# actapia/rna_clique

Hardware: AMD Instinct MI355X
Metric: sample-pairs/sec (all-vs-all alignment -> RBH graph -> distance matrix) (higher is better)
Workload: dtype u8/int32

## Files before the change

### include/rcgpu.h

```cpp
#ifndef RCGPU_H
#define RCGPU_H

#include <stdint.h>

#ifdef __cplusplus
extern "C" {
#endif

#define RC_OK 0
#define RC_E_ARG (-1)
#define RC_E_STATE (-2)
#define RC_E_HIP (-3)
#define RC_E_NOMEM (-4)
#define RC_E_NO_IDEAL (-5)
#define RC_E_CAPACITY (-6)
#define RC_E_LIMIT (-7)
#define RC_E_IO (-8)

typedef struct rc_engine rc_engine;

typedef struct rc_opts {
    int32_t top_matches;
    int32_t keep_all;
    double evalue;
// ... 66 lines not shown
    double dev_peak_bytes;
    double defer_length;
    double defer_gaveup;
    double defer_outside;
    double index_reused;
    double ext_retries;
    double load_ms;
    double align_wall_ms;
    double host_wait_ms;
    double later_seeds;
    double later_whole;
    double index_fb_ranges;
    double index_fb_keys;
    double resample_ms;
    double nj_ms;
} rc_timing;

void rc_default_opts(rc_opts *opts);

int rc_create(const rc_opts *opts, rc_engine **eng);
int rc_destroy(rc_engine *eng);
const char *rc_last_error(void);
void rc_dev_peak_reset(void);

int rc_add_sample(rc_engine *eng, const char *label, const char *seq,
                  const uint64_t *tx_offsets, const int32_t *gene,
                  const int32_t *iso, uint32_t n_tx, int32_t *sample_id);

int rc_add_hsps(rc_engine *eng, int32_t q, int32_t s, const rc_hsp *hsps, uint64_t n);

int rc_upload(rc_engine *eng);

int rc_run(rc_engine *eng);
int rc_align(rc_engine *eng);
int rc_finish(rc_engine *eng);

uint64_t rc_edge_record_size(void);
int rc_export_edges(rc_engine *eng, void *buf, uint64_t cap, uint64_t *n, int on_device);
// ... 75 lines not shown
```

### rna_clique_amd/_native.py

```python
from __future__ import annotations

import ctypes
import os
import sys

import numpy as np

HERE = os.path.dirname(os.path.abspath(__file__))
LIB_PATH = os.environ.get("RC_LIB") or os.path.join(HERE, "librcgpu.so")

RC_OK = 0
RC_E_ARG = -1
RC_E_STATE = -2
RC_E_HIP = -3
RC_E_NOMEM = -4
RC_E_NO_IDEAL = -5
RC_E_CAPACITY = -6
RC_E_LIMIT = -7


class RcOpts(ctypes.Structure):
    _fields_ = [("top_matches", ctypes.c_int32), ("keep_all", ctypes.c_int32),
                ("evalue", ctypes.c_double), ("word_size", ctypes.c_int32),
                ("xdrop_half", ctypes.c_int32), ("device", ctypes.c_int32),
# ... 43 lines not shown

EDGE_RECORD_DTYPE = np.dtype([("a", np.uint32), ("b", np.uint32), ("pair", np.uint32),
                              ("nident", np.int32), ("den", np.int32)])
RC_EDGE_SUM_ONLY = 0x80000000
RC_NODE_ONLY = 0x7FFFFFFF


class RcTiming(ctypes.Structure):
    _fields_ = [(n, ctypes.c_double) for n in (
        "pack_ms", "index_ms", "align_ms", "topn_ms", "rbh_ms", "graph_ms",
        "reduce_ms", "total_ms", "seed_kernel_ms", "align_kernel_ms", "ext_steps",
        "ext_calls", "ext_fullband", "ext_deferred", "big_passes", "tiles", "dust_ms",
        "band_bound", "maxhsp_bound", "ext_second", "near_index", "reverse_seeds", "ext_slides", "ext_wide", "dev_bytes",
        "dev_peak_bytes", "defer_length", "defer_gaveup", "defer_outside", "index_reused",
        "ext_retries", "load_ms", "align_wall_ms", "host_wait_ms", "later_seeds", "later_whole",
        "index_fb_ranges", "index_fb_keys", "resample_ms", "nj_ms")]


assert HSP_DTYPE.itemsize == ctypes.sizeof(RcHsp)
assert ROW_DTYPE.itemsize == ctypes.sizeof(RcRow)

P = ctypes.POINTER
VP = ctypes.c_void_p
SIGNATURES = {
    "rc_default_opts": (None, [P(RcOpts)]),
    "rc_create": (ctypes.c_int, [P(RcOpts), P(VP)]),
    "rc_destroy": (ctypes.c_int, [VP]),
    "rc_last_error": (ctypes.c_char_p, []),
    "rc_dev_peak_reset": (None, []),
    "rc_add_sample": (ctypes.c_int, [VP, ctypes.c_char_p, ctypes.c_char_p,
                                     P(ctypes.c_uint64), P(ctypes.c_int32),
                                     P(ctypes.c_int32), ctypes.c_uint32,
                                     P(ctypes.c_int32)]),
    "rc_add_hsps": (ctypes.c_int, [VP, ctypes.c_int32, ctypes.c_int32, VP, ctypes.c_uint64]),
    "rc_upload": (ctypes.c_int, [VP]),
    "rc_run": (ctypes.c_int, [VP]),
    "rc_align": (ctypes.c_int, [VP]),
    "rc_finish": (ctypes.c_int, [VP]),
    "rc_edge_record_size": (ctypes.c_uint64, []),
    "rc_export_edges": (ctypes.c_int, [VP, VP, ctypes.c_uint64, P(ctypes.c_uint64), ctypes.c_int]),
    "rc_import_edges": (ctypes.c_int, [VP, VP, ctypes.c_uint64, ctypes.c_int]),
    "rc_import_edge_parts": (ctypes.c_int, [VP, VP, VP, ctypes.c_int32, ctypes.c_uint64, ctypes.c_int]),
    "rc_trim": (ctypes.c_int, [VP]),
    "rc_set_sample_count": (ctypes.c_int, [VP, ctypes.c_int32]),
# ... 78 lines not shown
```

### rna_clique_amd/csrc/align.hip

```cpp
#include "device.h"

#include <algorithm>
#include <climits>
#include <cstdlib>
#include <type_traits>

namespace rcg {

constexpr int SBLOCK = 256;
#ifndef RC_SEED_CAP
#define RC_SEED_CAP 512
#endif
#ifndef RC_SEED_WAVES
#define RC_SEED_WAVES 5
#endif
constexpr int SEED_CAP = RC_SEED_CAP;
static_assert((SEED_CAP & (SEED_CAP - 1)) == 0, "RC_SEED_CAP must be a power of two");
#ifndef RC_HBATCH
#define RC_HBATCH 6
#endif
constexpr int HBATCH = RC_HBATCH;
#ifndef RC_SEED_REV_WAVES
#define RC_SEED_REV_WAVES 7
#endif
// ... 1431 lines not shown
__device__ __forceinline__ RowArgsK row_args()
{
    RowArgsK p = (RowArgsK)__builtin_amdgcn_kernarg_segment_ptr();
    asm volatile("" : "+s"(p));
    return p;
}

struct RowLds {
    int meta[RM_N];
    int st[RS_N];
};
enum { WM_GA0, WM_GB0, WM_AARR, WM_BARR, WM_ALO, WM_ALIM, WM_BLO, WM_BLIM, WM_W0, WM_N = WM_W0 + 4 };
struct RowWin {
    int w[WM_N];
};
__host__ __device__ constexpr size_t row_lds_bytes(int rw, int na, int sw, bool win = false)
{
    return ((size_t)(EBLOCK / rw) * na * sw + 2) * 8 + (NSHARD + 1) * 8 + (size_t)(EBLOCK / rw) * sizeof(RowLds) + 32 +
           (win ? (size_t)(EBLOCK / rw) * sizeof(RowWin) : 0);
}
constexpr int WIN_MARGIN = 48;

template <bool AMB, int RW, int MINW, bool SAVE = false, bool WIN = false>
__global__ __launch_bounds__(EBLOCK, MINW) void extend_rows_kernel(RowArgs)
{
    constexpr int RROWS = EBLOCK / RW;
    constexpr int RC0 = RW / 2;
    constexpr int NA = AMB ? 8 : 4;
    constexpr int EBIT = 26, OBIT = 13;
    extern __shared__ uint64_t rstg[];
    const int sw = row_args()->P.dsw;
    unsigned long long *const sprefix = reinterpret_cast<unsigned long long *>(rstg + 2 + (size_t)RROWS * NA * sw);
    RowLds *const rows_lds = reinterpret_cast<RowLds *>(sprefix + NSHARD + 1);
    uint32_t *const rcnt = reinterpret_cast<uint32_t *>(rows_lds + RROWS);
    uint32_t &s_ncand = rcnt[4];
    RowWin *const rows_win = reinterpret_cast<RowWin *>(rcnt + 8);
    {
        const RowArgsK K = row_args();
        if (threadIdx.x < 4 || threadIdx.x == 5) rcnt[threadIdx.x] = 0;
        for (int i = threadIdx.x; i <= NSHARD; i += EBLOCK) sprefix[i] = K->P.shard_prefix[i];
        if (threadIdx.x == 0) s_ncand = K->P.list ? (uint32_t)*K->P.list_n : (uint32_t)K->P.n_cand;
    }
    __syncthreads();

    const int lane = threadIdx.x & 63, rl = lane & (RW - 1), row = lane / RW;
    const int rs = threadIdx.x / RW;
    const int k = rl - RC0;
    uint64_t *stg = rstg + 2 + (size_t)rs * NA * sw;
    const uint32_t base0 = 4u * (uint32_t)reinterpret_cast<uintptr_t>(rstg) + (uint32_t)(2 + rs * NA * sw) * 32u;
    const uint32_t bqr = base0 + 64u * (uint32_t)sw, btr = bqr + 32u * (uint32_t)sw;
    const uint32_t moff = 128u * (uint32_t)sw;
    RowLds &RL = rows_lds[rs];
    int *meta = RL.meta;
    int *const wm = rows_win[rs].w;
    const int X = row_args()->P.xdrop;
    auto chunk = []() { return (uint32_t)max(row_args()->P.chunk, 1); };
    uint32_t lnx = 0;
    auto grab = [&]() {
        const uint32_t ncand = s_ncand, ch = chunk();
        unsigned long long b = 0;
        if (rl == 0) b = atomicAdd(row_args()->P.work, (unsigned long long)ch);
        b = (unsigned long long)__shfl((long long)b, RW * row);
        lnx = b < ncand ? (uint32_t)b : ncand;
        if (rl == 0) RL.st[RS_LEND] = (int)(lnx + ch);
    };
    auto slot = [&](uint32_t l, int which) -> uint64_t {
        int sh = RL.st[which];
        while (sh + 1 < NSHARD && sprefix[sh + 1] <= l) sh++;
        if (rl == 0) RL.st[which] = sh;
// ... 21 lines not shown
            } else if (wide && K->P.wide) {
                wi2 = atomicAdd(K->P.wide_n, 1ull);
                K->P.wide[wi2] = (uint32_t)ci;
            }
            box_out()[ci * BOX_REC + FX_STATUS] = -1;
        }
        if constexpr (SAVE) return (unsigned long long)__shfl((long long)wi2, RW * row);
        return wi2;
    };
    if (rl == 0) {
        RL.st[RS_SHARD] = 0;
        RL.st[RS_SHN] = 0;
    }
    grab();
    int recv = load_rec(lnx);

    int act = A_FETCH;
    int R = -1, goe = 0, wi = 0, wg = 0, wd = 0, best = 0, bl = RC0, d6 = 0;
    uint32_t pa = 0, pb = 0;
    int alen = 0, blen = 0;
    uint32_t pbk = 0;
    int blk = 0, nkd = 0;
    int mnk = 0;
    bool swap = false;
    int wlo = 0, wlim = 0;

    using GW = const __attribute__((address_space(1))) uint64_t *;
    auto warr = [](int arr, bool mask) -> GW {
        const RowArgsK K = row_args();
        GW f = (GW)(mask ? K->db.AF : K->db.F), r = (GW)(mask ? K->db.ARC : K->db.RC);
// ... 106 lines not shown
#endif
        int r0 = 0;
        if constexpr (WIN) {
            win_begin(done_act == A_LDONE ? 1 : 0);
            const int m0 = min(alen, blen);
            bool pend = false;
            if (rl == RC0) {
                const int mw = min(m0, wlim);
                r0 = slide_fwd<AMB>(pa, pb, max(mw, 0), moff);
                pend = mw < m0 && r0 >= mw;
            }
            if (ballot(pend)) win_resolve(0, r0, m0, pend);
        } else {
            if (rl == RC0) r0 = slide_fwd<AMB>(pa, pb, min(alen, blen), moff);
        }
        r0 = __shfl(r0, RW * row + RC0);
        best = 2 * r0;
        bl = RC0;
        if (rl == RC0) {
            wi = r0;
            wg = 0;
            wd = 0;
        }
        R = rl == RC0 ? r0 : -1;
        goe = 0;
        if (rl == 0 && d6) atomicAdd(&rcnt[5], (uint32_t)d6);
        d6 = 0;
        if constexpr (!WIN) pbk = pb - (uint32_t)k;
        blk = blen + k;
        mnk = max(min(alen, blk), 0);
        nkd = -k;
        if (rl == 0) {
            atomicAdd(&rcnt[0], 1u);
            meta[RM_PHASE] = done_act;
            meta[RM_KOF] = 0;
        }
        act = (min(alen, blen) - r0 <= 0) ? done_act : done_act + (A_STEP_R - A_RDONE);
#ifdef RC_ROW_TIMING
        t_ei += __builtin_readcyclecounter() - e0t;
#endif
    };

#ifdef RC_ROW_TIMING
    unsigned long long t_tr = 0, t_st = 0, t_fe = 0, t_sl = 0;
    unsigned long long n16 = 0, c16 = 0, sl16 = 0;
    bool ov16 = false, had = false;
    int w16 = 0;
#endif
    for (;;) {
#ifdef RC_ROW_TIMING
        const unsigned long long c0t = __builtin_readcyclecounter();
#endif
        while (act < A_DONE) {
            if (act == A_FETCH) {
#ifdef RC_ROW_TIMING
                const unsigned long long f0t = __builtin_readcyclecounter();
#endif
                if (lnx >= s_ncand) {
                    R = -1;
                    act = A_DONE;
                    continue;
                }
                const uint64_t ci = cslot(lnx, RS_SHARD);
#ifdef RC_ROW_TIMING
                if (rl == 0 && had && !ov16) c16++;
                ov16 = false;
                had = true;
#endif
                if (rl < CAND_DWORDS) meta[RM_REC + rl] = recv;
                if (rl == 0) {
                    meta[RM_CLO] = (int)(uint32_t)ci;
                    meta[RM_CHI] = (int)(uint32_t)(ci >> 32);
// ... 191 lines not shown
                    }
                    bl = BL_PARKED;
                }
                const int from = rl + s;
                const bool in = from >= 0 && from < RW;
                const int nR = __shfl(R, RW * row + (in ? from : rl)), ng = __shfl(goe, RW * row + (in ? from : rl));
                R = in ? nR : -1;
                goe = in ? ng : 0;
                pbk -= (uint32_t)s;
                blk += s;
                mnk = max(min(alen, blk), 0);
                nkd -= s;
                if constexpr (WIN) win_lane(k + kn);
                if (rl == 0) {
                    meta[RM_KOF] = kn;
                    atomicAdd(&rcnt[3], 1u);
                }
                __builtin_amdgcn_fence(__ATOMIC_RELEASE, "wavefront");
                __builtin_amdgcn_wave_barrier();
                act = meta[RM_PHASE] + (A_STEP_R - A_RDONE);
#ifdef RC_ROW_TIMING
                t_sl += __builtin_readcyclecounter() - s0t;
#endif
            } else if (act == A_RDONE || act == A_LDONE) {
                int ei, ed, ego, kb;
                if (bl == BL_PARKED) {
                    ei = meta[RM_PWI];
                    ed = meta[RM_PWD] / 6;
                    ego = meta[RM_PWG];
                    kb = meta[RM_PK];
                } else {
// ... 13 lines not shown
                        meta[RM_RI] = ei;
                        meta[RM_RJ] = ej;
                        meta[RM_RD] = ed;
                        meta[RM_RGO] = ego;
                    }
                    const int x = meta[RM_X], y = meta[RM_Y];
                    const int Lq = meta[RM_REC + RC_LQ], Lt = meta[RM_REC + RC_LT];
                    pa = (uint32_t)meta[RM_QB] + (uint32_t)(Lq - x);
                    alen = x;
                    pb = (uint32_t)meta[RM_TB] + (uint32_t)(Lt - y);
                    blen = y;
                    if (swap) {
                        const uint32_t t = pa; pa = pb; pb = t;
                        const int u = alen; alen = blen; blen = u;
                    }
                    ext_init(A_LDONE);
                } else {
                    const uint64_t ci = (uint64_t)(uint32_t)meta[RM_CLO] | ((uint64_t)(uint32_t)meta[RM_CHI] << 32);
                    int v = 0;
                    if (rl >= FX_R && rl < FX_R + 5) v = meta[RM_RSC + (rl - FX_R)];
                    if (rl == FX_L) v = best;
                    if (rl == FX_L + 1) v = ei;
                    if (rl == FX_L + 2) v = ej;
                    if (rl == FX_L + 3) v = ed;
                    if (rl == FX_L + 4) v = ego;
                    if (rl < BOX_REC) box_out()[ci * BOX_REC + rl] = v;
                    act = A_FETCH;
                }
            } else {
                const uint64_t ci = (uint64_t)(uint32_t)meta[RM_CLO] | ((uint64_t)(uint32_t)meta[RM_CHI] << 32);
                const unsigned long long wi2 = defer(ci, true);
                if constexpr (SAVE && RW == 32) {
                    if (wi2 != ~0ull) {
                        const RowArgsK K = row_args();
                        if (K->P.resume && wi2 < K->P.res_cap) {
                            int *rec = K->P.resume + (size_t)wi2 * RES_REC;
                            rec[RES_R + rl] = R;
                            rec[RES_G + rl] = goe;
                            if (rl <= RES_PK) rec[rl] = meta[RM_RSC + rl];
                            if (rl == RES_D6) rec[rl] = meta[RM_AD6];
                            if (rl == RES_BEST) rec[rl] = meta[RM_ABEST];
                        }
                    }
                }
                if (rl == 0) atomicAdd(&rcnt[2], 1u);
                act = A_FETCH;
            }
        }
#ifdef RC_ROW_TIMING
        const unsigned long long c1t = __builtin_readcyclecounter();
        t_tr += c1t - c0t;
#endif
        const bool ext = act >= A_STEP_R;
        const uint64_t mext = m_ge(act, A_STEP_R);
        if (!mext) break;
        if (ext) {
            d6 += 6;
            nkd -= 6;
            const int Rl = rw_from_lower<RW, true>(R, -1, rl), Rr = rw_from_upper<RW, true>(R, -1, rl);
            const int gl = rw_from_lower<RW, false>(goe, 0, rl), gr = rw_from_upper<RW, false>(goe, 0, rl);
// ... 86 lines not shown
            const uint64_t medge = RW == 64 ? 0ull : rw_spread<RW>(mlive & EDGES);
            act = lane_sel(mcont, lane_sel_k<A_SLIDE>(medge, act), act - (A_STEP_R - A_RDONE));
        }
#ifdef RC_ROW_TIMING
        t_st += __builtin_readcyclecounter() - c1t;
#endif
    }
#ifdef RC_ROW_TIMING
    unsigned long long *const counters = row_args()->P.counters;
    if (lane == 0 && counters) {
        atomicAdd(&counters[DC_T_TRANS - DC_COUNTERS], t_tr);
        atomicAdd(&counters[DC_T_STEPS - DC_COUNTERS], t_st);
        atomicAdd(&counters[DC_T_FETCH - DC_COUNTERS], t_fe);
        atomicAdd(&counters[DC_T_SLIDE - DC_COUNTERS], t_sl);
        atomicAdd(&counters[DC_T_START - DC_COUNTERS], t_ei);
    }
    if (rl == 0 && had && !ov16) c16++;
    if (rl == 0 && counters) {
        atomicAdd(&counters[DC_T_N16 - DC_COUNTERS], n16);
        atomicAdd(&counters[DC_T_C16 - DC_COUNTERS], c16);
        atomicAdd(&counters[DC_T_SL16 - DC_COUNTERS], sl16);
    }
#endif
    unsigned long long *const ctr = row_args()->P.counters;
    if (rl == 0 && d6) atomicAdd(&rcnt[5], (uint32_t)d6);
    __syncthreads();
    if (threadIdx.x < 4 && ctr) atomicAdd(&ctr[DC_EXTS - DC_COUNTERS + threadIdx.x], (unsigned long long)rcnt[threadIdx.x]);
    if (threadIdx.x == 5 && ctr) atomicAdd(&ctr[DC_STEPS - DC_COUNTERS], (unsigned long long)(rcnt[5] / 6u));
}

__global__ __launch_bounds__(256) void first_finish_kernel(ExtParams P)
{
    constexpr int OBIT = 13, GMASK = 8191;
    for (uint64_t li = blockIdx.x * (uint64_t)blockDim.x + threadIdx.x; li < P.n_cand;
         li += (uint64_t)gridDim.x * blockDim.x) {
        int lo = 0, hi = NSHARD;
        while (hi - lo > 1) {
            const int mid = (lo + hi) >> 1;
            if (P.shard_prefix[mid] <= li) lo = mid; else hi = mid;
        }
        const uint64_t ci = (uint64_t)lo * P.cand_cap + (li - P.shard_prefix[lo]);
// ... 572 lines not shown
    if (hipOccupancyMaxActiveBlocksPerMultiprocessor(&per_cu, kernel, EBLOCK, lds) != hipSuccess || per_cu < 1)
        per_cu = 1;
    return (unsigned)(cus * per_cu);
}

template <bool A, int RWV, bool SV, bool WV>
static void launch_rows_t(const Db &db, const ExtParams &P, hipStream_t st)
{
    auto kern = extend_rows_kernel<A, RWV, ROW_MIN_WAVES, SV, WV>;
    const size_t lds = row_lds_bytes(RWV, A ? 8 : 4, P.dsw, WV);
    hipLaunchKernelGGL(kern, dim3(resident_blocks(kern, lds)), dim3(EBLOCK), lds, st, RowArgs{db, P});
}
template <int RWV, bool SV = false>
static void launch_rows(bool amb, const Db &db, const ExtParams &P, hipStream_t st)
{
    if (amb) {
        if (P.win) launch_rows_t<true, RWV, SV, true>(db, P, st); else launch_rows_t<true, RWV, SV, false>(db, P, st);
    } else {
        if (P.win) launch_rows_t<false, RWV, SV, true>(db, P, st); else launch_rows_t<false, RWV, SV, false>(db, P, st);
    }
}

int row_slot_words_max(bool amb)
{
    const int na = amb ? 8 : 4, rows = EBLOCK / 32;
    const size_t per_block = (size_t)(160 * 1024) / (size_t)ROW_MIN_WAVES;
    const size_t fixed = row_lds_bytes(32, na, 0, true);
    return (int)((per_block - fixed) / ((size_t)rows * na * 8));
}

static void extend_lists(bool amb, const Db &db, const ExtParams &B, hipStream_t st)
{
    for (int dir = 0; dir < (B.share ? 2 : 1); dir++) {
        ExtParams W3 = B;
        W3.dir = dir;
        if (dir) {
            W3.defer = B.defer_r;
            W3.defer_count = B.defer_r_count;
        }
        if (amb) {
            auto kern = extend_kernel<true>;
            hipLaunchKernelGGL(kern, dim3(resident_blocks(kern, 0)), dim3(EBLOCK), 0, st, db, W3);
        } else {
// ... 147 lines not shown
```

### rna_clique_amd/csrc/device.h

```cpp
#pragma once
#include <hip/hip_runtime.h>
#include <stdint.h>

namespace rcg {

constexpr int W16 = 16;
constexpr int BAND = 64;
constexpr int BAND_LO = -32;
constexpr int MAX_HSP = 8;
constexpr int DMAX = 4096;
constexpr int ISO_LDS = 128;
constexpr uint64_t MAX_TX = 1ull << 27;
constexpr int MAX_SAMPLES = 65535;

struct TxInfo {
    uint64_t start;
    uint32_t len;
    int32_t sample;
};

__host__ __device__ __forceinline__ size_t grp_index(uint32_t gene, int sample, uint32_t n_genes)
{
    return (size_t)sample * n_genes + gene;
}
// ... 194 lines not shown
    DC_DEFER_R,
    DC_WORK3,
    DC_MBIG,
    DC_WIDE0,
    DC_WIDE1,
    DC_WORK_W0,
    DC_WORK_W1,
    DC_WHY,
    DC_WHY_END = DC_WHY + 3,
    DC_T_N16 = DC_WHY_END,
    DC_T_FETCH,
    DC_T_SLIDE,
    DC_T_START,
    DC_T_C16,
    DC_T_SL16,
    DC_N = 32
};
static_assert(DC_DEFER == DC_COUNTERS + 5 && DC_WORK == DC_COUNTERS + 6, "defer_count and work alias counters[5], [6]");
static_assert(DC_COUNTERS_END == 12 && DC_WHY == 22 && DC_T_SL16 == 30 && DC_T_SL16 < DC_N, "d_count layout");

struct ExtParams {
    int32_t xdrop;
    int32_t sym;
    int32_t max_len;
    const int32_t *thr;
    const int32_t *bits10;
    const Cand *cands;
    const GSeed *seeds;
    const unsigned long long *shard_prefix;
    uint64_t n_cand;
    uint64_t cand_cap;
    DHsp *cand_hsp;
    uint8_t *cand_nh;
    uint32_t *cand_ovf;
    DHsp *ovf;
    uint64_t ovf_cap;
    unsigned long long *ovf_count;
    unsigned int *status;
    unsigned long long *counters;
    int32_t dsw;
    int32_t win;
    int32_t *cand_box;
    int32_t chunk;
    unsigned long long *work;
    uint32_t *defer;
    unsigned long long *defer_count;
    const uint32_t *list;
    const unsigned long long *list_n;
    int32_t share;
    int32_t which;
    int32_t dir;
    int32_t *cand_box2;
    DHsp *cand_hsp_r;
    uint8_t *cand_nh_r;
    uint32_t *cand_ovf_r;
    uint32_t *defer_r;
// ... 180 lines not shown
```

### rna_clique_amd/csrc/engine.hip

```cpp
#include "../../include/rcgpu.h"
#include "device.h"
#include "graph_pickle.h"

#include <cstring>
#include <rocprim/device/device_radix_sort.hpp>
#include <rocprim/device/device_scan.hpp>
#include <rocprim/iterator/counting_iterator.hpp>

#include <algorithm>
#include <cmath>
#include <cstdio>
#include <cstdlib>
#include <cstring>
#include <array>
#include <atomic>
#include <chrono>
#include <condition_variable>
#include <deque>
#include <functional>
#include <map>
#include <memory>
#include <mutex>
#include <numeric>
#include <string>
// ... 42 lines not shown
void launch_near_fill(bool, const TxInfo *, uint32_t, const uint8_t *, const uint64_t *, const uint64_t *,
                      const uint64_t *, uint64_t *, uint64_t, unsigned long long *, hipStream_t);
void launch_seed(bool, const Db &, const Index &, const SeedParams &, hipStream_t);
void launch_seed_big(bool, const Db &, const Index &, const SeedParams &, uint32_t, hipStream_t);
void launch_rs_range(const uint32_t *, uint32_t, uint32_t, uint32_t, uint32_t *, hipStream_t);
void launch_dust(bool, uint64_t, uint64_t, const uint64_t *, const uint64_t *, const uint64_t *, const TxInfo *, uint32_t, int,
                 int, int, uint32_t *, uint64_t *, uint32_t, uint64_t *, hipStream_t);
uint32_t dust_scratch_words(uint32_t);
uint64_t dust_event_words(uint32_t);
void launch_extend_rows(bool, const Db &, const ExtParams &, hipStream_t);
void launch_extend_retry(bool, const Db &, const ExtParams &, hipStream_t);
void launch_later_rounds(bool, const Db &, const ExtParams &, bool, const LaterParams &, Cand *const[2],
                         uint32_t *const[2], int32_t *const[2], uint32_t *const[2], unsigned long long *, hipStream_t);
void launch_later_finish(const ExtParams &, const LaterParams &, hipStream_t);
int row_slot_words_max(bool amb);
void launch_group(const GroupParams &, int, hipStream_t);

void launch_rbh(const RbhParams &, int, hipStream_t);
void launch_hkey(const DHsp *h, uint64_t n, const uint32_t *tx_gene, HKey *out, hipStream_t st);
void launch_rbh_place(const RbhParams &, hipStream_t);
void launch_gather_rows(const DHsp *, const DRow *, uint64_t, DHsp *, hipStream_t);
void launch_cc(const DEdge *, uint64_t, uint32_t, const int32_t *, int, int, uint32_t *, uint32_t *, uint32_t *,
               uint32_t *, uint32_t *, uint8_t *, unsigned long long *, hipStream_t);
void launch_pair_sums(const DEdge *, uint64_t, const uint32_t *, const uint8_t *, unsigned long long *,
                      unsigned long long *, unsigned long long *, unsigned long long *, hipStream_t);
void launch_distance(const unsigned long long *, const unsigned long long *, const int32_t *, const int32_t *,
                     int, int, double *, unsigned int *, hipStream_t);
void launch_comp_keys(const uint32_t *, const uint32_t *, const uint8_t *, const uint32_t *, uint32_t, uint64_t *,
                      unsigned long long *, hipStream_t);
void launch_comp_members(const uint64_t *, uint64_t, uint32_t, uint32_t *, unsigned long long *, hipStream_t);
// ... 196 lines not shown
static const uint64_t TILE_ALIGN = 1ull << POS_TX_SHIFT;
static uint64_t align_up(uint64_t x) { return (x + TILE_ALIGN - 1) & ~(TILE_ALIGN - 1); }

struct Knobs {
    bool share;
    uint64_t tile_bases;
    bool tile_split;
    int ovf_cap0;
    int win_words;
    bool later;
    int later_rows;
    uint64_t later_cap;
    bool rbh_two_pass;
    int resume;
    uint32_t index_cap;
    int nj_lds;
};

static Knobs read_knobs()
{
    const auto env = [](const char *name) -> const char * { return getenv(name); };
    const auto num = [&](const char *name, int unset) { return env(name) ? atoi(env(name)) : unset; };
    Knobs k{};
    k.share = num("RC_SHARE", 1) != 0;
    k.tile_bases = env("RC_TILE_BASES") ? std::max<uint64_t>(strtoull(env("RC_TILE_BASES"), nullptr, 10), TILE_ALIGN)
                                        : (1ull << 32) - (1ull << 24);
    k.tile_split = num("RC_TILE_SPLIT", 1) != 0;
    k.ovf_cap0 = env("RC_OVF_CAP0") ? std::max(1, num("RC_OVF_CAP0", 1)) : 0;
    k.win_words = env("RC_WIN_WORDS") ? std::max(4, num("RC_WIN_WORDS", 4)) : 0;
    k.later = num("RC_LATER", 1) != 0;
    k.later_rows = num("RC_LATER_ROWS", 64);
    k.later_cap = env("RC_LATER_CAP") ? (uint64_t)std::max(atoll(env("RC_LATER_CAP")), 1ll) : (24ull << 20);
    k.rbh_two_pass = env("RC_RBH_TWO_PASS") != nullptr;
    k.resume = num("RC_RESUME", -1);
    k.index_cap = env("RC_INDEX_CAP") ? (uint32_t)std::max(2, num("RC_INDEX_CAP", 2)) : 0u;
    k.nj_lds = std::min(128, std::max(0, num("RC_NJ_LDS", 128)));
    return k;
}

struct rc_engine {
    rc_opts o{};
    Knobs knobs{};
    hipStream_t st = nullptr;
    hipStream_t st2 = nullptr;
    std::vector<SampleRec> samples;
    uint64_t total_bases = 0;
    uint64_t ascii_used = 0;
    std::vector<uint64_t> tx_start{0};
    std::vector<int32_t> tx_sample, tx_gene_id, tx_iso;
    bool has_amb = false;
// ... 184 lines not shown
    o->word_size = 28;
    o->xdrop_half = 108;
    o->device = 0;
    o->shard_rank = 0;
    o->shard_count = 1;
    o->symmetric = 0;
    o->dust_level = 20;
    o->dust_window = 64;
    o->dust_linker = 1;
}

const char *rc_last_error(void) { return g_err.c_str(); }

void rc_dev_peak_reset(void) { g_dev_peak.store(g_dev_bytes.load()); }

uint64_t rc_edge_record_size(void) { return sizeof(DEdge); }

int rc_create(const rc_opts *opts, rc_engine **out)
{
    if (!opts || !out) return fail(RC_E_ARG, "null argument");
    if (opts->top_matches < 1) return fail(RC_E_ARG, "top_matches must be >= 1");
    if (opts->word_size < W16 || opts->word_size > 64) return fail(RC_E_ARG, "word_size must be in [16, 64]");
    if (opts->xdrop_half < 0) return fail(RC_E_ARG, "xdrop_half must be >= 0");
    if (opts->dust_level < 0 || (opts->dust_level > 0 && (opts->dust_window < 8 || opts->dust_window > 64 ||
                                                          opts->dust_linker < 0)))
        return fail(RC_E_ARG, "bad DUST parameters");
    if (opts->dust_level > 0 && opts->symmetric)
        return fail(RC_E_ARG, "DUST masks each direction's query: it needs symmetric = 0");
    if (opts->shard_count < 1 || opts->shard_rank < 0 || opts->shard_rank >= opts->shard_count)
        return fail(RC_E_ARG, "bad shard");
// ... 1266 lines not shown
    X.cand_cap = e->cand_cap;
    X.cand_hsp = e->d_cand_hsp.p;
    X.cand_nh = e->d_cand_nh.p;
    X.cand_ovf = e->d_cand_ovf.p;
    X.ovf = e->d_ovf.p;
    X.ovf_cap = e->ovf_cap;
    X.ovf_count = cnt + DC_OVF;
    X.status = e->d_status.p;
    X.counters = cnt + DC_COUNTERS;
    {
        const int need = ((e->max_len + 31) >> 5) + 4;
        const int smax = row_slot_words_max(e->has_amb);
        const int forced = e->knobs.win_words;
        X.win = forced ? 1 : (need > smax ? 1 : 0);
        X.dsw = forced ? std::min(forced, smax) : std::min(need, smax);
    }
    X.defer = e->d_defer.p;
    X.defer_count = cnt + DC_DEFER;
    X.work = cnt + DC_WORK;
    X.cand_box = e->d_cand_box.p;
    X.share = e->share ? 1 : 0;
    X.which = 0;
    X.dir = 0;
    X.cand_box2 = e->d_cand_box2.p;
    X.cand_hsp_r = e->d_cand_hsp_r.p;
    X.cand_nh_r = e->d_cand_nh_r.p;
    X.cand_ovf_r = e->d_cand_ovf_r.p;
    X.defer_r = e->d_defer_r.p;
    X.defer_r_count = cnt + DC_DEFER_R;
    X.list2 = e->d_list2.p;
// ... 101 lines not shown
        CHK(e->d_wide0.ensure(std::max<uint64_t>(n_cand, 1)));
        CHK(e->d_wide1.ensure(std::max<uint64_t>(n_cand, 1)));
        e->res_cap = e->knobs.resume == 0 ? 0u : (uint32_t)std::min<uint64_t>(n_cand, 12u << 20);
        if (e->knobs.resume != 1 && e->ovf_frac <= 0.02) e->res_cap = 0;
        if (e->res_cap) CHK(e->d_resume.ensure((size_t)e->res_cap * RES_REC));
    }
    CHK(e->d_defer.ensure(std::max<uint64_t>(n_cand, 1)));
    C.later_on = false;
    for (int attempt = 0;; attempt++) {
        if (attempt == 4) return fail(RC_E_NOMEM, "HSP overflow buffer kept overflowing");
        CHK(e->d_ovf.ensure(e->ovf_cap));
        if (attempt == 0) {
            HIPCHK(hipMemsetAsync(cnt + DC_OVF, 0, (DC_COUNTERS_END - DC_OVF) * sizeof(unsigned long long), e->st));
            HIPCHK(hipMemsetAsync(cnt + DC_DEFER_R, 0, (DC_MBIG - DC_DEFER_R) * sizeof(unsigned long long), e->st));
            HIPCHK(hipMemsetAsync(cnt + DC_WIDE0, 0, (DC_WHY_END - DC_WIDE0) * sizeof(unsigned long long), e->st));
        } else {
            HIPCHK(hipMemsetAsync(cnt + DC_OVF, 0, sizeof(unsigned long long), e->st));
        }
        HIPCHK(hipMemsetAsync(e->d_status.p, 0, 4 * sizeof(unsigned int), e->st));
        ExtParams X = ext_params(e, C);
        if (attempt == 0) {
            HIPCHK(hipEventRecord(e->ev[10], e->st));
            launch_extend_rows(e->has_amb, C.db, X, e->st);
            HIPCHK(hipGetLastError());
            unsigned long long dn[2] = {0, 0};
            HIPCHK(hipMemcpyAsync(&dn[0], X.defer_count, sizeof dn[0], hipMemcpyDeviceToHost, e->st));
            HIPCHK(hipMemcpyAsync(&dn[1], X.defer_r_count, sizeof dn[1], hipMemcpyDeviceToHost, e->st));
            CHK(wait_st(e));
            const uint64_t nd = dn[0] + dn[1];
            const uint64_t want = std::min<uint64_t>(2 * nd, (uint64_t)(MAX_HSP - 1) * nd) + 1024;
// ... 17 lines not shown
            e->tm.ext_retries += 1.0;
        }
        launch_extend_retry(e->has_amb, C.db, X, e->st);
        HIPCHK(hipGetLastError());
        HIPCHK(hipEventRecord(e->ev[11], e->st));
        unsigned long long ovn = 0, ctr[DC_COUNTERS_END - DC_COUNTERS] = {};
        const auto c = [&](int slot) { return (double)ctr[slot - DC_COUNTERS]; };
        unsigned long long nwide[2] = {0, 0};
        static_assert(DC_WIDE1 == DC_WIDE0 + 1, "read together");
        HIPCHK(hipMemcpyAsync(nwide, cnt + DC_WIDE0, sizeof nwide, hipMemcpyDeviceToHost, e->st));
        unsigned long long why[DC_WHY_END - DC_WHY] = {0, 0, 0};
        HIPCHK(hipMemcpyAsync(why, cnt + DC_WHY, sizeof why, hipMemcpyDeviceToHost, e->st));
        unsigned long long ndr = 0, nl2 = 0;
        HIPCHK(hipMemcpyAsync(&ndr, cnt + DC_DEFER_R, sizeof ndr, hipMemcpyDeviceToHost, e->st));
        HIPCHK(hipMemcpyAsync(&nl2, cnt + DC_LIST2, sizeof nl2, hipMemcpyDeviceToHost, e->st));
        unsigned int status = 0;
        HIPCHK(hipMemcpyAsync(&ovn, cnt + DC_OVF, sizeof ovn, hipMemcpyDeviceToHost, e->st));
        HIPCHK(hipMemcpyAsync(ctr, cnt + DC_COUNTERS, sizeof ctr, hipMemcpyDeviceToHost, e->st));
        HIPCHK(hipMemcpyAsync(&status, e->d_status.p, sizeof status, hipMemcpyDeviceToHost, e->st));
        CHK(wait_st(e));
        if (c(DC_T_TRANS) || c(DC_T_STEPS)) CHK(print_row_timing(e, ctr));
        if (!(status & 1u)) {
            e->tm.ext_steps += c(DC_STEPS);
            e->tm.ext_calls += c(DC_EXTS);
            e->tm.ext_fullband += c(DC_FULLBAND);
            e->ovf_frac = n_cand ? c(DC_FULLBAND) / (double)n_cand : 0.0;
            e->tm.ext_deferred += c(DC_DEFER) + (double)ndr;
            e->tm.ext_second += e->share ? (double)nl2 : 0.0;
            e->tm.band_bound += c(DC_BAND_BOUND);
            e->tm.ext_slides += c(DC_SLIDES);
            e->tm.ext_wide += (double)(nwide[0] + nwide[1]);
            e->tm.maxhsp_bound += c(DC_MAXHSP);
            e->tm.defer_length += (double)why[0];
            e->tm.defer_gaveup += (double)why[1];
            e->tm.defer_outside += (double)why[2];
            if (C.later_on) {
                std::vector<unsigned long long> lc((size_t)MAX_HSP * LATER_CNT + LC_N);
                HIPCHK(hipMemcpy(lc.data(), e->d_lcnt.p, lc.size() * sizeof(unsigned long long),
                                 hipMemcpyDeviceToHost));
                for (int r = 0; r < MAX_HSP; r++) e->tm.later_seeds += (double)lc[(size_t)r * LATER_CNT];
                e->tm.later_whole += (double)lc[(size_t)MAX_HSP * LATER_CNT + LC_WHOLE];
            }
            break;
        }
        e->ovf_cap = std::max<uint64_t>(e->ovf_cap, ovn * 5 / 4 + 1024);
// ... 1611 lines not shown
```

Before: 2385.

## Prefetch next candidate's sequences into LDS in the row extension kernel

Adds a prefetching variant of the row extension kernel for 32-lane rows without ambiguity masks or windows. It double-buffers the forward query/subject slices and seed record for the next candidate via global_load_lds while the current candidate extends, and replaces per-event LDS atomics with per-row counters flushed at the end. The goal is to hide global-memory latency at candidate fetch. In exchange it uses more LDS per block, which may lower occupancy, and adds waitcnt synchronisation complexity.

After: 2397 (median of 6 runs). Within noise of the previous version (+0.5%).

```diff
diff --git a/include/rcgpu.h b/include/rcgpu.h
--- a/include/rcgpu.h
+++ b/include/rcgpu.h
@@ -104,6 +104,7 @@
     double index_fb_keys;
     double resample_ms;
     double nj_ms;
+    double ext_prefetched;
 } rc_timing;
 
 void rc_default_opts(rc_opts *opts);
@@ -112,6 +113,7 @@
 int rc_destroy(rc_engine *eng);
 const char *rc_last_error(void);
 void rc_dev_peak_reset(void);
+int rc_row_prefetch_words(int32_t max_len);
 
 int rc_add_sample(rc_engine *eng, const char *label, const char *seq,
                   const uint64_t *tx_offsets, const int32_t *gene,
diff --git a/rna_clique_amd/_native.py b/rna_clique_amd/_native.py
--- a/rna_clique_amd/_native.py
+++ b/rna_clique_amd/_native.py
@@ -81,7 +81,7 @@
         "band_bound", "maxhsp_bound", "ext_second", "near_index", "reverse_seeds", "ext_slides", "ext_wide", "dev_bytes",
         "dev_peak_bytes", "defer_length", "defer_gaveup", "defer_outside", "index_reused",
         "ext_retries", "load_ms", "align_wall_ms", "host_wait_ms", "later_seeds", "later_whole",
-        "index_fb_ranges", "index_fb_keys", "resample_ms", "nj_ms")]
+        "index_fb_ranges", "index_fb_keys", "resample_ms", "nj_ms", "ext_prefetched")]
 
 
 assert HSP_DTYPE.itemsize == ctypes.sizeof(RcHsp)
@@ -95,6 +95,7 @@
     "rc_destroy": (ctypes.c_int, [VP]),
     "rc_last_error": (ctypes.c_char_p, []),
     "rc_dev_peak_reset": (None, []),
+    "rc_row_prefetch_words": (ctypes.c_int, [ctypes.c_int32]),
     "rc_add_sample": (ctypes.c_int, [VP, ctypes.c_char_p, ctypes.c_char_p,
                                      P(ctypes.c_uint64), P(ctypes.c_int32),
                                      P(ctypes.c_int32), ctypes.c_uint32,
diff --git a/rna_clique_amd/csrc/align.hip b/rna_clique_amd/csrc/align.hip
--- a/rna_clique_amd/csrc/align.hip
+++ b/rna_clique_amd/csrc/align.hip
@@ -1469,22 +1469,30 @@
 struct RowWin {
     int w[WM_N];
 };
-__host__ __device__ constexpr size_t row_lds_bytes(int rw, int na, int sw, bool win = false)
+enum { PF_REC = 0, PF_L = CAND_DWORDS, PF_FLAG, PF_PAR, PF_SEED = CAND_DWORDS + 4,
+       PF_CNT = PF_SEED + 8, PC_EXT = 0, PC_CAND, PC_OVF, PC_SLIDE, PC_STEP6, PC_PF, PC_N, PF_N = PF_CNT + PC_N };
+struct RowPf {
+    int w[sizeof(RowLds) / 4];
+};
+static_assert(PF_SEED % 4 == 0 && PF_N <= (int)(sizeof(RowLds) / 4), "RowPf layout");
+constexpr int PF_SLOTS = 6;
+__host__ __device__ constexpr size_t row_lds_bytes(int rw, int na, int sw, bool win = false, bool pf = false)
 {
     return ((size_t)(EBLOCK / rw) * na * sw + 2) * 8 + (NSHARD + 1) * 8 + (size_t)(EBLOCK / rw) * sizeof(RowLds) + 32 +
-           (win ? (size_t)(EBLOCK / rw) * sizeof(RowWin) : 0);
+           (win ? (size_t)(EBLOCK / rw) * sizeof(RowWin) : 0) + (pf ? (size_t)(EBLOCK / rw) * sizeof(RowPf) : 0);
 }
 constexpr int WIN_MARGIN = 48;
 
-template <bool AMB, int RW, int MINW, bool SAVE = false, bool WIN = false>
+template <bool AMB, int RW, int MINW, bool SAVE = false, bool WIN = false, bool PF = false>
 __global__ __launch_bounds__(EBLOCK, MINW) void extend_rows_kernel(RowArgs)
 {
+    static_assert(!PF || (RW == 32 && !AMB && !WIN), "six-array staging: 32-lane rows, whole transcripts, no masks");
     constexpr int RROWS = EBLOCK / RW;
     constexpr int RC0 = RW / 2;
-    constexpr int NA = AMB ? 8 : 4;
+    constexpr int NA = PF ? PF_SLOTS : (AMB ? 8 : 4);
     constexpr int EBIT = 26, OBIT = 13;
     extern __shared__ uint64_t rstg[];
-    const int sw = row_args()->P.dsw;
+    const int sw = PF ? row_args()->P.dsw6 : row_args()->P.dsw;
     unsigned long long *const sprefix = reinterpret_cast<unsigned long long *>(rstg + 2 + (size_t)RROWS * NA * sw);
     RowLds *const rows_lds = reinterpret_cast<RowLds *>(sprefix + NSHARD + 1);
     uint32_t *const rcnt = reinterpret_cast<uint32_t *>(rows_lds + RROWS);
@@ -1492,7 +1500,7 @@
     RowWin *const rows_win = reinterpret_cast<RowWin *>(rcnt + 8);
     {
         const RowArgsK K = row_args();
-        if (threadIdx.x < 4 || threadIdx.x == 5) rcnt[threadIdx.x] = 0;
+        if (threadIdx.x < 4 || threadIdx.x == 5 || threadIdx.x == 6) rcnt[threadIdx.x] = 0;
         for (int i = threadIdx.x; i <= NSHARD; i += EBLOCK) sprefix[i] = K->P.shard_prefix[i];
         if (threadIdx.x == 0) s_ncand = K->P.list ? (uint32_t)*K->P.list_n : (uint32_t)K->P.n_cand;
     }
@@ -1508,6 +1516,10 @@
     RowLds &RL = rows_lds[rs];
     int *meta = RL.meta;
     int *const wm = rows_win[rs].w;
+    int *const pf = meta + (RROWS * (int)(sizeof(RowLds) / 4) + 8);
+    auto count = [&](int which, uint32_t v) {
+        if constexpr (PF) pf[PF_CNT + which] += (int)v; else atomicAdd(&rcnt[which], v);
+    };
     const int X = row_args()->P.xdrop;
     auto chunk = []() { return (uint32_t)max(row_args()->P.chunk, 1); };
     uint32_t lnx = 0;
@@ -1559,6 +1571,31 @@
     }
     grab();
     int recv = load_rec(lnx);
+#ifdef RC_ROW_TIMING
+    unsigned long long t_pw = 0;
+#endif
+    auto pf_wait = [&]() {
+#ifdef RC_ROW_TIMING
+        const unsigned long long w0t = __builtin_readcyclecounter();
+#endif
+        asm volatile("s_waitcnt vmcnt(0)" ::: "memory");
+#ifdef RC_ROW_TIMING
+        t_pw += __builtin_readcyclecounter() - w0t;
+#endif
+    };
+    if constexpr (PF) {
+        if (rl < CAND_DWORDS) pf[PF_REC + rl] = recv;
+        if (rl == 0) {
+            pf[PF_L] = (int)lnx;
+            pf[PF_FLAG] = 0;
+            pf[PF_PAR] = 0;
+            for (int i = 0; i < PC_N; i++) pf[PF_CNT + i] = 0;
+        }
+        if (++lnx >= (uint32_t)RL.st[RS_LEND]) grab();
+        recv = load_rec(lnx);
+        __builtin_amdgcn_fence(__ATOMIC_RELEASE, "wavefront");
+        __builtin_amdgcn_wave_barrier();
+    }
 
     int act = A_FETCH;
     int R = -1, goe = 0, wi = 0, wg = 0, wd = 0, best = 0, bl = RC0, d6 = 0;
@@ -1695,7 +1732,13 @@
         } else {
             if (rl == RC0) r0 = slide_fwd<AMB>(pa, pb, min(alen, blen), moff);
         }
-        r0 = __shfl(r0, RW * row + RC0);
+        if constexpr (PF) {
+            int ro = row;
+            asm volatile("" : "+v"(ro));
+            r0 = __shfl(r0, RW * ro + RC0);
+        } else {
+            r0 = __shfl(r0, RW * row + RC0);
+        }
         best = 2 * r0;
         bl = RC0;
         if (rl == RC0) {
@@ -1705,14 +1748,14 @@
         }
         R = rl == RC0 ? r0 : -1;
         goe = 0;
-        if (rl == 0 && d6) atomicAdd(&rcnt[5], (uint32_t)d6);
+        if (rl == 0 && d6) count(PF ? PC_STEP6 : 5, (uint32_t)d6);
         d6 = 0;
         if constexpr (!WIN) pbk = pb - (uint32_t)k;
         blk = blen + k;
         mnk = max(min(alen, blk), 0);
         nkd = -k;
         if (rl == 0) {
-            atomicAdd(&rcnt[0], 1u);
+            count(0, 1u);
             meta[RM_PHASE] = done_act;
             meta[RM_KOF] = 0;
         }
@@ -1737,6 +1780,125 @@
 #ifdef RC_ROW_TIMING
                 const unsigned long long f0t = __builtin_readcyclecounter();
 #endif
+                if constexpr (PF) {
+                    using GV = const __attribute__((address_space(1))) void *;
+                    using GD = const __attribute__((address_space(1))) uint32_t *;
+                    using LP = __attribute__((address_space(3))) void *;
+                    int lc[3] = {rl, row, rs};
+                    asm volatile("" : "+v"(lc[0]), "+v"(lc[1]), "+v"(lc[2]));
+                    const int rl = lc[0], row = lc[1], rs = lc[2];
+                    const int sw = row_args()->P.dsw6;
+                    const uint32_t l = (uint32_t)pf[PF_L];
+                    if (l >= s_ncand) {
+                        R = -1;
+                        act = A_DONE;
+                        continue;
+                    }
+                    const uint64_t ci = cslot(l, RS_SHARD);
+#ifdef RC_ROW_TIMING
+                    if (rl == 0 && had && !ov16) c16++;
+                    ov16 = false;
+                    had = true;
+#endif
+                    const int flag = pf[PF_FLAG], par = pf[PF_PAR];
+                    pf_wait();
+                    const int crec = rl < CAND_DWORDS ? pf[PF_REC + rl] : 0;
+                    if (rl < CAND_DWORDS) {
+                        meta[RM_REC + rl] = crec;
+                        pf[PF_REC + rl] = recv;
+                    }
+                    if (rl == 0) {
+                        meta[RM_CLO] = (int)(uint32_t)ci;
+                        meta[RM_CHI] = (int)(uint32_t)(ci >> 32);
+                        pf[PF_L] = (int)lnx;
+                    }
+                    if (++lnx >= (uint32_t)RL.st[RS_LEND]) grab();
+                    recv = load_rec(lnx);
+                    __builtin_amdgcn_fence(__ATOMIC_RELEASE, "wavefront");
+                    __builtin_amdgcn_wave_barrier();
+                    const RowArgsK K = row_args();
+                    const uint32_t total = (uint32_t)K->db.total;
+                    auto stage = [&](bool mine, GW arr, uint32_t g0, int L, uint32_t dstb) {
+                        const int c = min((int)(((g0 & 63u) + (uint32_t)L) >> 5) + 3, sw);
+                        const GW src = arr + ((g0 >> 5) & ~1u) + 2 * rl;
+                        if (mine && 2 * rl < c)
+                            __builtin_amdgcn_global_load_lds((GV)src, (LP)(uintptr_t)(dstb - (uint32_t)row * (RW * 16u)), 16, 0,
+                                                             0);
+                    };
+                    auto stage_seed = [&](bool mine, uint32_t soff, uint32_t e01, uint32_t dstb) {
+                        const GD sp = (GD)(K->P.seeds + (soff + (K->P.which ? e01 >> 16 : e01 & 0xFFFFu))) + rl;
+                        if (mine && rl < 3)
+                            __builtin_amdgcn_global_load_lds((GV)sp, (LP)(uintptr_t)(dstb - (uint32_t)row * (RW * 4u)), 4, 0, 0);
+                    };
+                    const int Lq = meta[RM_REC + RC_LQ], Lt = meta[RM_REC + RC_LT];
+                    const uint32_t q0 = (uint32_t)meta[RM_REC + RC_Q0], s0 = (uint32_t)meta[RM_REC + RC_S0];
+                    const int strand = (meta[RM_REC + RC_CNT_STRAND] >> 16) & 1;
+                    const uint32_t rq0 = total - q0 - (uint32_t)Lq, rs0 = total - s0 - (uint32_t)Lt;
+                    GW dF = (GW)K->db.F, dRC = (GW)K->db.RC;
+                    asm volatile("" : "+s"(dF), "+s"(dRC));
+                    const uint32_t sb = (uint32_t)reinterpret_cast<uintptr_t>(rstg) + (uint32_t)(2 + rs * NA * sw) * 8u;
+                    const uint32_t fb = sb + (par ? 32u * (uint32_t)sw : 0u), nb = sb + (par ? 0u : 32u * (uint32_t)sw);
+                    const uint32_t sdb = (uint32_t)reinterpret_cast<uintptr_t>(pf + PF_SEED);
+                    const int nLq = pf[PF_REC + RC_LQ], nLt = pf[PF_REC + RC_LT];
+                    const uint32_t nq0 = (uint32_t)pf[PF_REC + RC_Q0], ns0 = (uint32_t)pf[PF_REC + RC_S0];
+                    const int nstrand = (pf[PF_REC + RC_CNT_STRAND] >> 16) & 1;
+                    const bool nf = (uint32_t)pf[PF_L] < s_ncand;
+                    auto issue = [&](bool mine) {
+                        if (!flag) {
+                            stage(mine, strand ? dRC : dF, q0, Lq, fb);
+                            stage(mine, dF, s0, Lt, fb + 8u * (uint32_t)sw);
+                            stage_seed(mine, (uint32_t)meta[RM_REC + RC_SOFF], (uint32_t)meta[RM_REC + RC_E01],
+                                       sdb + 16u * (uint32_t)par);
+                        }
+                        stage(mine, strand ? dF : dRC, rq0, Lq, sb + 16u * (uint32_t)sw);
+                        stage(mine, dRC, rs0, Lt, sb + 24u * (uint32_t)sw);
+                        if (nf) {
+                            stage(mine, nstrand ? dRC : dF, nq0, nLq, nb);
+                            stage(mine, dF, ns0, nLt, nb + 8u * (uint32_t)sw);
+                            stage_seed(mine, (uint32_t)pf[PF_REC + RC_SOFF], (uint32_t)pf[PF_REC + RC_E01],
+                                       sdb + 16u * (uint32_t)(par ^ 1));
+                        }
+                    };
+                    const uint64_t fm = ballot(true);
+                    if ((uint32_t)fm && (uint32_t)(fm >> 32)) {
+                        issue(row == 0);
+                        issue(row == 1);
+                    } else {
+                        issue(true);
+                    }
+                    if (rl == 0) {
+                        pf[PF_FLAG] = nf ? 1 : 0;
+                        pf[PF_PAR] = par ^ 1;
+                        pf[PF_CNT + PC_PF] += flag;
+                        pf[PF_CNT + PC_CAND] += 1;
+                        meta[RM_QB] = (int)(4u * sb + 64u * (uint32_t)sw + (rq0 & 63u));
+                        meta[RM_TB] = (int)(4u * sb + 96u * (uint32_t)sw + (rs0 & 63u));
+                    }
+                    if (!flag) pf_wait();
+                    if (rl == 0) {
+                        meta[RM_X] = pf[PF_SEED + 4 * par];
+                        meta[RM_Y] = pf[PF_SEED + 4 * par + 1];
+                        meta[RM_LEN] = (int)((uint32_t)pf[PF_SEED + 4 * par + 2] & SEED_LEN);
+                    }
+                    __builtin_amdgcn_fence(__ATOMIC_RELEASE, "wavefront");
+                    __builtin_amdgcn_wave_barrier();
+                    const int x = meta[RM_X], y = meta[RM_Y], len = meta[RM_LEN];
+                    const uint32_t sams = (uint32_t)meta[RM_REC + RC_SAMS];
+                    swap = (sams & 0xFFFFu) > (sams >> 16);
+                    pa = 4u * fb + (q0 & 63u) + (uint32_t)(x + len);
+                    alen = Lq - (x + len);
+                    pb = 4u * fb + 32u * (uint32_t)sw + (s0 & 63u) + (uint32_t)(y + len);
+                    blen = Lt - (y + len);
+                    if (swap) {
+                        const uint32_t t = pa; pa = pb; pb = t;
+                        const int u = alen; alen = blen; blen = u;
+                    }
+                    ext_init(A_RDONE);
+#ifdef RC_ROW_TIMING
+                    t_fe += __builtin_readcyclecounter() - f0t;
+#endif
+                    continue;
+                }
                 if (lnx >= s_ncand) {
                     R = -1;
                     act = A_DONE;
@@ -1958,7 +2120,7 @@
                 if constexpr (WIN) win_lane(k + kn);
                 if (rl == 0) {
                     meta[RM_KOF] = kn;
-                    atomicAdd(&rcnt[3], 1u);
+                    count(3, 1u);
                 }
                 __builtin_amdgcn_fence(__ATOMIC_RELEASE, "wavefront");
                 __builtin_amdgcn_wave_barrier();
@@ -2002,10 +2164,13 @@
                         const uint32_t t = pa; pa = pb; pb = t;
                         const int u = alen; alen = blen; blen = u;
                     }
+                    if constexpr (PF) pf_wait();
                     ext_init(A_LDONE);
                 } else {
                     const uint64_t ci = (uint64_t)(uint32_t)meta[RM_CLO] | ((uint64_t)(uint32_t)meta[RM_CHI] << 32);
                     int v = 0;
+                    int rl = k + RC0;
+                    if constexpr (PF) asm volatile("" : "+v"(rl));
                     if (rl >= FX_R && rl < FX_R + 5) v = meta[RM_RSC + (rl - FX_R)];
                     if (rl == FX_L) v = best;
                     if (rl == FX_L + 1) v = ei;
@@ -2031,7 +2196,7 @@
                         }
                     }
                 }
-                if (rl == 0) atomicAdd(&rcnt[2], 1u);
+                if (rl == 0) count(2, 1u);
                 act = A_FETCH;
             }
         }
@@ -2148,6 +2313,7 @@
         atomicAdd(&counters[DC_T_FETCH - DC_COUNTERS], t_fe);
         atomicAdd(&counters[DC_T_SLIDE - DC_COUNTERS], t_sl);
         atomicAdd(&counters[DC_T_START - DC_COUNTERS], t_ei);
+        if (PF) atomicAdd(&counters[DC_T_PFWAIT - DC_COUNTERS], t_pw);
     }
     if (rl == 0 && had && !ov16) c16++;
     if (rl == 0 && counters) {
@@ -2158,7 +2324,16 @@
 #endif
     unsigned long long *const ctr = row_args()->P.counters;
     if (rl == 0 && d6) atomicAdd(&rcnt[5], (uint32_t)d6);
+    if constexpr (PF) {
+        asm volatile("s_waitcnt vmcnt(0)" ::: "memory");
+        if (rl == 0) {
+            for (int i = 0; i < 4; i++) atomicAdd(&rcnt[i], (uint32_t)pf[PF_CNT + i]);
+            atomicAdd(&rcnt[5], (uint32_t)pf[PF_CNT + PC_STEP6]);
+            atomicAdd(&rcnt[6], (uint32_t)pf[PF_CNT + PC_PF]);
+        }
+    }
     __syncthreads();
+    if (PF && threadIdx.x == 6 && ctr) atomicAdd(&ctr[DC_PREFETCHED - DC_COUNTERS], (unsigned long long)rcnt[6]);
     if (threadIdx.x < 4 && ctr) atomicAdd(&ctr[DC_EXTS - DC_COUNTERS + threadIdx.x], (unsigned long long)rcnt[threadIdx.x]);
     if (threadIdx.x == 5 && ctr) atomicAdd(&ctr[DC_STEPS - DC_COUNTERS], (unsigned long long)(rcnt[5] / 6u));
 }
@@ -2761,6 +2936,14 @@
 template <int RWV, bool SV = false>
 static void launch_rows(bool amb, const Db &db, const ExtParams &P, hipStream_t st)
 {
+    if constexpr (RWV == 32) {
+        if (!amb && !P.win && P.dsw6) {
+            auto kern = extend_rows_kernel<false, 32, ROW_MIN_WAVES, SV, false, true>;
+            const size_t lds = row_lds_bytes(32, PF_SLOTS, P.dsw6, false, true);
+            hipLaunchKernelGGL(kern, dim3(resident_blocks(kern, lds)), dim3(EBLOCK), lds, st, RowArgs{db, P});
+            return;
+        }
+    }
     if (amb) {
         if (P.win) launch_rows_t<true, RWV, SV, true>(db, P, st); else launch_rows_t<true, RWV, SV, false>(db, P, st);
     } else {
@@ -2774,6 +2957,14 @@
     const size_t per_block = (size_t)(160 * 1024) / (size_t)ROW_MIN_WAVES;
     const size_t fixed = row_lds_bytes(32, na, 0, true);
     return (int)((per_block - fixed) / ((size_t)rows * na * 8));
+}
+
+int row_prefetch_words(int max_len)
+{
+    const int need = ((max_len + 31) >> 5) + 4;
+    const int sw = std::max(12, (need + 1) & ~1);
+    const size_t per_block = (size_t)(160 * 1024) / (size_t)ROW_MIN_WAVES;
+    return row_lds_bytes(32, PF_SLOTS, sw, false, true) <= per_block ? sw : 0;
 }
 
 static void extend_lists(bool amb, const Db &db, const ExtParams &B, hipStream_t st)
diff --git a/rna_clique_amd/csrc/device.h b/rna_clique_amd/csrc/device.h
--- a/rna_clique_amd/csrc/device.h
+++ b/rna_clique_amd/csrc/device.h
@@ -232,10 +232,13 @@
     DC_T_START,
     DC_T_C16,
     DC_T_SL16,
-    DC_N = 32
+    DC_PREFETCHED,
+    DC_T_PFWAIT,
+    DC_N = 40
 };
 static_assert(DC_DEFER == DC_COUNTERS + 5 && DC_WORK == DC_COUNTERS + 6, "defer_count and work alias counters[5], [6]");
-static_assert(DC_COUNTERS_END == 12 && DC_WHY == 22 && DC_T_SL16 == 30 && DC_T_SL16 < DC_N, "d_count layout");
+static_assert(DC_COUNTERS_END == 12 && DC_WHY == 22 && DC_T_SL16 == 30 && DC_T_PFWAIT == 32 && DC_T_PFWAIT < DC_N,
+              "d_count layout");
 
 struct ExtParams {
     int32_t xdrop;
@@ -258,6 +261,7 @@
     unsigned long long *counters;
     int32_t dsw;
     int32_t win;
+    int32_t dsw6;
     int32_t *cand_box;
     int32_t chunk;
     unsigned long long *work;
diff --git a/rna_clique_amd/csrc/engine.hip b/rna_clique_amd/csrc/engine.hip
--- a/rna_clique_amd/csrc/engine.hip
+++ b/rna_clique_amd/csrc/engine.hip
@@ -80,6 +80,7 @@
                          uint32_t *const[2], int32_t *const[2], uint32_t *const[2], unsigned long long *, hipStream_t);
 void launch_later_finish(const ExtParams &, const LaterParams &, hipStream_t);
 int row_slot_words_max(bool amb);
+int row_prefetch_words(int max_len);
 void launch_group(const GroupParams &, int, hipStream_t);
 
 void launch_rbh(const RbhParams &, int, hipStream_t);
@@ -306,6 +307,7 @@
     bool rbh_two_pass;
     int resume;
     uint32_t index_cap;
+    bool row_prefetch;
     int nj_lds;
 };
 
@@ -326,6 +328,7 @@
     k.rbh_two_pass = env("RC_RBH_TWO_PASS") != nullptr;
     k.resume = num("RC_RESUME", -1);
     k.index_cap = env("RC_INDEX_CAP") ? (uint32_t)std::max(2, num("RC_INDEX_CAP", 2)) : 0u;
+    k.row_prefetch = num("RC_ROW_PREFETCH", 1) != 0;
     k.nj_lds = std::min(128, std::max(0, num("RC_NJ_LDS", 128)));
     return k;
 }
@@ -540,6 +543,8 @@
 
 void rc_dev_peak_reset(void) { g_dev_peak.store(g_dev_bytes.load()); }
 
+int rc_row_prefetch_words(int32_t max_len) { return max_len < 0 ? 0 : row_prefetch_words(max_len); }
+
 uint64_t rc_edge_record_size(void) { return sizeof(DEdge); }
 
 int rc_create(const rc_opts *opts, rc_engine **out)
@@ -1836,6 +1841,7 @@
         const int forced = e->knobs.win_words;
         X.win = forced ? 1 : (need > smax ? 1 : 0);
         X.dsw = forced ? std::min(forced, smax) : std::min(need, smax);
+        X.dsw6 = e->knobs.row_prefetch && !X.win && !e->has_amb ? row_prefetch_words(e->max_len) : 0;
     }
     X.defer = e->d_defer.p;
     X.defer_count = cnt + DC_DEFER;
@@ -1967,6 +1973,7 @@
             HIPCHK(hipMemsetAsync(cnt + DC_OVF, 0, (DC_COUNTERS_END - DC_OVF) * sizeof(unsigned long long), e->st));
             HIPCHK(hipMemsetAsync(cnt + DC_DEFER_R, 0, (DC_MBIG - DC_DEFER_R) * sizeof(unsigned long long), e->st));
             HIPCHK(hipMemsetAsync(cnt + DC_WIDE0, 0, (DC_WHY_END - DC_WIDE0) * sizeof(unsigned long long), e->st));
+            HIPCHK(hipMemsetAsync(cnt + DC_PREFETCHED, 0, (DC_N - DC_PREFETCHED) * sizeof(unsigned long long), e->st));
         } else {
             HIPCHK(hipMemsetAsync(cnt + DC_OVF, 0, sizeof(unsigned long long), e->st));
         }
@@ -2014,12 +2021,18 @@
         unsigned long long ndr = 0, nl2 = 0;
         HIPCHK(hipMemcpyAsync(&ndr, cnt + DC_DEFER_R, sizeof ndr, hipMemcpyDeviceToHost, e->st));
         HIPCHK(hipMemcpyAsync(&nl2, cnt + DC_LIST2, sizeof nl2, hipMemcpyDeviceToHost, e->st));
+        unsigned long long npf[2] = {0, 0};
+        static_assert(DC_T_PFWAIT == DC_PREFETCHED + 1, "read together");
+        HIPCHK(hipMemcpyAsync(npf, cnt + DC_PREFETCHED, sizeof npf, hipMemcpyDeviceToHost, e->st));
         unsigned int status = 0;
         HIPCHK(hipMemcpyAsync(&ovn, cnt + DC_OVF, sizeof ovn, hipMemcpyDeviceToHost, e->st));
         HIPCHK(hipMemcpyAsync(ctr, cnt + DC_COUNTERS, sizeof ctr, hipMemcpyDeviceToHost, e->st));
         HIPCHK(hipMemcpyAsync(&status, e->d_status.p, sizeof status, hipMemcpyDeviceToHost, e->st));
         CHK(wait_st(e));
-        if (c(DC_T_TRANS) || c(DC_T_STEPS)) CHK(print_row_timing(e, ctr));
+        if (c(DC_T_TRANS) || c(DC_T_STEPS)) {
+            CHK(print_row_timing(e, ctr));
+            fprintf(stderr, "row kernel wave-cycles waiting for prefetched loads %.4g\n", (double)npf[1]);
+        }
         if (!(status & 1u)) {
             e->tm.ext_steps += c(DC_STEPS);
             e->tm.ext_calls += c(DC_EXTS);
@@ -2029,6 +2042,7 @@
             e->tm.ext_second += e->share ? (double)nl2 : 0.0;
             e->tm.band_bound += c(DC_BAND_BOUND);
             e->tm.ext_slides += c(DC_SLIDES);
+            e->tm.ext_prefetched += (double)npf[0];
             e->tm.ext_wide += (double)(nwide[0] + nwide[1]);
             e->tm.maxhsp_bound += c(DC_MAXHSP);
             e->tm.defer_length += (double)why[0];
```
